# 54rt1n/shardmerge

Hardware: AMD Instinct MI355X
Metric: merged-weight GB/s per GPU + % HBM roofline, Llama-3-70B 3-way FFT merge (higher is better)
Workload: dtype f32; 1 GPU; Llama-3-70B block tensors, this rank's 1/8 slice (9 per block x 10 blocks), K=3 finetunes, bf16 in/out, resident in HBM; workload_id=llama3-70b-slice, k=3, parallelism=tensor-partition x1 (no data-path collective), streams_per_gpu=8

## Files before the change

shardmerge_amd/csrc/fft_engine.hpp:

```cpp
#pragma once
#include <cmath>
#include <cstdint>
#include <type_traits>

#if defined(__HIPCC__)
#include <hip/hip_runtime.h>
#define SM_HD __host__ __device__ __forceinline__
#else
#define SM_HD inline
#endif
#define SM_CONST static constexpr
#if defined(__HIP_DEVICE_COMPILE__)
#define SM_OPAQUE(x) asm volatile("" : "+v"(x))
#else
#define SM_OPAQUE(x) ((void)0)
#endif
#if defined(__HIP_DEVICE_COMPILE__)
#define SM_LAUNDER(x) asm("" : "+v"(x))
#else
#define SM_LAUNDER(x) ((void)0)
#endif
#if defined(__HIP_DEVICE_COMPILE__) && !defined(SM_NO_SCHED_BARRIER)
#define SM_SCHED_FENCE() __builtin_amdgcn_sched_barrier(0)
#else
// ... 548 lines not shown
                    im[i] = mk2(xi[m * R + i], xi[(m + 1) * R + i]);
                }
                if (Ns > 1) apply_twiddles<R>(re, im, tw, (j0 % Ns) * tstep, (j1 % Ns) * tstep);
                Dft<R>::run(re, im);
#pragma unroll
                for (int i = 0; i < R; ++i) {
                    xr[m * R + i] = re[i].x; xr[(m + 1) * R + i] = re[i].y;
                    xi[m * R + i] = im[i].x; xi[(m + 1) * R + i] = im[i].y;
                }
            }
        }
    } else {
#pragma unroll
        for (int m = 0; m < MB; ++m) {
            const int j = t + m * T;
            if (j < nb) {
                if (Ns > 1) {
                    const int k = j % Ns;
                    if constexpr (R <= 32 && R != 28) {
                        apply_twiddles<R>(xr + m * R, xi + m * R, tw, k * tstep, 0);
                    } else {
#pragma unroll
                        for (int i = 1; i < R; ++i) {
                            const cf2 w = tw[i * k * tstep];
                            cmul(xr[m * R + i], xi[m * R + i], w.x, w.y);
                        }
                    }
                }
                if constexpr (R == 32 && PACK == 0) DftComposite<4, 8>::run(xr + m * R, xi + m * R);
                else Dft<R>::run(xr + m * R, xi + m * R);
            }
        }
    }
}

template <int COMP, class S> SM_HD float* comp_of(S& s) { if constexpr (COMP == 0) return s.xr; else return s.xi; }

struct DynPlan { static constexpr bool is_static = false; static constexpr bool cx = false; static constexpr int waves = 4; };
template <int N_, int T_, bool CX_, int WAVES_, int... RS>
struct SPlan {
    static constexpr bool is_static = true;
    static constexpr bool cx = false;
    static constexpr int waves = WAVES_;
    static constexpr int N = N_, T = T_, npass = (int)sizeof...(RS);
    static constexpr int radix(int i) { constexpr int r[] = {RS...}; return r[i]; }
    static constexpr int ns(int p) { int v = 1; for (int i = 0; i < p; ++i) v *= radix(i); return v; }
    static constexpr int lds_floats = ((N_ + (N_ >> 5) + 1 + 31) / 32) * 32;
    static_assert(ns(npass) == N_, "radices must multiply to N");
};
template <class P> SM_HD int plan_N(const FftPlanDev& pl) { if constexpr (P::is_static) return P::N; else return pl.N; }
template <class P> SM_HD int plan_T(const FftPlanDev& pl) { if constexpr (P::is_static) return P::T; else return pl.T; }
template <class P> SM_HD int plan_lds(const FftPlanDev& pl) { if constexpr (P::is_static) return P::lds_floats; else return pl.lds_floats; }

#ifndef SM_DIAG_NOFFT
#define SM_DIAG_NOFFT 0
#endif
struct FloatPairRef { float& a; float& b; };
struct NoHook { template <class C> SM_HD void operator()(C) const {} };
template <class P, int PACK = 1, int DIAG = 0, int SKIPS = 0, class Ex, class StT, class NatScatter, class FinGather, class AfterNat = NoHook>
SM_HD void wg_fft(Ex& ex, StT& st, const FftPlanDev& pl, float* lds, NatScatter nat_scatter, FinGather fin_gather, AfterNat after_nat = AfterNat{}) {
    using S = typename StT::value_type;
    const int N = plan_N<P>(pl), T = plan_T<P>(pl), LF = plan_lds<P>(pl);
    if constexpr ((SM_DIAG_NOFFT & DIAG) != 0) {
        static_for<0, 2>([&](auto comp_c) {
            ex.each(st, [&](int tid, S& s) { nat_scatter(tid, s, comp_c); });
            ex.sync();
// ... 91 lines not shown
```

shardmerge_amd/csrc/sm_aten_core.hpp:

```cpp
#pragma once
#include <cmath>
#include <cstring>

#include "fft_engine.hpp"

namespace smhip {

SM_HD float aten_u2f(uint32_t u) { float f; memcpy(&f, &u, 4); return f; }
SM_HD uint32_t aten_f2u(float f) { uint32_t u; memcpy(&u, &f, 4); return u; }

constexpr int ATEN_LANES = 8;
constexpr int ATEN_THREADS = 256;
constexpr int ATEN_ROWS_PER_THREAD = 32;
constexpr int ATEN_CHUNK_ROWS = ATEN_THREADS * ATEN_ROWS_PER_THREAD;
constexpr int ATEN_MAX_SIGS = 16;
constexpr int ATEN_NO_EXP = -32768;

struct AtenSum { double A; uint32_t B0, B1p; };
SM_HD AtenSum aten_sum_identity() { AtenSum r; r.A = 0.0; r.B0 = 0u; r.B1p = 0u; return r; }
SM_HD AtenSum aten_sum_stop() { AtenSum r; r.A = INFINITY; r.B0 = 0u; r.B1p = 0u; return r; }
SM_HD AtenSum aten_compose(const AtenSum& l, const AtenSum& r) {
    const uint32_t pl = l.B1p >> 31, lb1 = l.B1p & 0x7fffffffu;
    const uint32_t pr = r.B1p >> 31, rb1 = r.B1p & 0x7fffffffu;
    const uint32_t mid0 = (pl ^ l.B0) & 1u, mid1 = (1u ^ pl ^ lb1) & 1u;
// ... 105 lines not shown
            constexpr int k0 = decltype(kb_c)::value * 8;
            float y[8];
#pragma unroll
            for (int k = 0; k < 8; ++k) y[k] = b[8 * (k0 + k) + ((k0 + k) >> 2)];
#pragma unroll
            for (int k = 0; k < 8; ++k) { aten_chain_add(s0, y[k]); aten_chain_add(s1, y[k]); }
            SM_SCHED_FENCE();
        });
        aten_d_of_chain(s0, ep, s.fd[0], s.fd[1]);
        aten_d_of_chain(s1, ep - 1, s.fd[2], s.fd[3]);
    });
    static_for<0, 3>([&](auto step_c) {
        constexpr int DELTA = 8 << decltype(step_c)::value;
        ex.template wave_shift_down<DELTA, 4>(st, [](S& s) { return (const uint32_t*)s.fd; }, [](S& s) { return (uint32_t*)s.fr; });
        ex.each(st, [&](int, S& s) {
            aten_d_compose(s.fd[0], s.fd[1], s.fr[0], s.fr[1]);
            aten_d_compose(s.fd[2], s.fd[3], s.fr[2], s.fr[3]);
        });
    });
    ex.each(st, [&](int tid, S& s) {
        int tid_ = tid;
        SM_OPAQUE(tid_);
        const int g = tid_ / T, t = tid_ % T;
        const int w = t >> 6, ln = t & 63;
        int sig = 0; long long mrow = 0;
        if (ln >= 8 || w >= NG || !where(g, sig, mrow)) return;
        const size_t G = (size_t)mrow * NG + w, chunk = G / ATEN_GROUPS;
        const size_t slot = ((size_t)(af.sig0 + sig) * af.nchunks + chunk) * 8 + ln;
        af.grp[(slot * 2 + 0) * ATEN_GROUPS + G % ATEN_GROUPS] = aten_sum_of_d(s.fd[0], s.fd[1]);
        af.grp[(slot * 2 + 1) * ATEN_GROUPS + G % ATEN_GROUPS] = aten_sum_of_d(s.fd[2], s.fd[3]);
    });
}

}
```

shardmerge_amd/csrc/sm_capi.inc:

```

struct smhip_ctx {
    smhip::Pipeline<SM_BACKEND> pipe;
    explicit smhip_ctx(int device) : pipe(device) {}
};

#define SM_GUARD(ctx)                      \
    if (!(ctx)) return SMHIP_ERR_ARG;      \
    (ctx)->pipe.err.clear();
#define SM_FINISH(ctx, rc)                                                        \
    do {                                                                          \
        int rc__ = (rc);                                                          \
        if (rc__ == SMHIP_OK && !(ctx)->pipe.be.ok()) {                           \
            (ctx)->pipe.err = (ctx)->pipe.be.error();                             \
            rc__ = SMHIP_ERR_HIP;                                                 \
        }                                                                         \
        return rc__;                                                              \
    } while (0)

extern "C" {

const char* smhip_version(void) { return SM_VERSION_STRING; }

int smhip_create(int device, smhip_ctx** out) {
    if (!out) return SMHIP_ERR_ARG;
// ... 170 lines not shown
    const int rc0 = ctx->pipe.reserve(1, 1);
    if (rc0) SM_FINISH(ctx, rc0);
    smhip::SigDesc sg{x, base, dtype, 1.f};
    double out = 0;
    if (!ctx->pipe.run_serial_norms(&sg, 1, n, &out))
        return ctx->pipe.fail(SMHIP_ERR_ARG, "reference_cpu norm: inputs must be 16-byte aligned");
    *norm_out = (float)out;
    SM_FINISH(ctx, SMHIP_OK);
}

int smhip_debug_option(smhip_ctx* ctx, const char* key, long value) {
    SM_GUARD(ctx);
    if (key && std::string(key) == "aten_overlap") { ctx->pipe.aten_overlap = value != 0; return SMHIP_OK; }
    if (key && std::string(key) == "emf_max_sample") { ctx->pipe.emf_max_sample = value >= 1 && value <= 4096 ? (int)value : smhip::EMF_MAX_SAMPLE; return SMHIP_OK; }
    if (key && std::string(key) == "aten_serial") { ctx->pipe.aten_serial = value != 0; return SMHIP_OK; }
    if (key && std::string(key) == "class_norms") { ctx->pipe.class_norms_mode = value >= 0 && value <= 2 ? (int)value : 1; return SMHIP_OK; }
    if (key && std::string(key) == "cand_cap") { ctx->pipe.debug_cand_cap = value > 0 ? (uint32_t)value : 0u; return SMHIP_OK; }
    if (key && std::string(key) == "sel_chunks") { ctx->pipe.debug_sel_chunks = value > 0 ? (uint32_t)value : 0u; return SMHIP_OK; }
    if (key && std::string(key) == "sel_flush_always") { ctx->pipe.debug_flush_always = value != 0; return SMHIP_OK; }
    if (key && std::string(key) == "fuse_norms") { ctx->pipe.fuse_norms = value != 0; return SMHIP_OK; }
    if (key && std::string(key) == "noise_seed") { ctx->pipe.noise_seed_base = (uint32_t)value; return SMHIP_OK; }
    if (key && std::string(key) == "spectral_intermediates") { ctx->pipe.spectral_inter = value != 0; return SMHIP_OK; }
    if (key && std::string(key) == "fuse_spec_norm") { ctx->pipe.fuse_spec_norm = value != 0; return SMHIP_OK; }
    if (key && std::string(key) == "sel_wgs_per_cu") { ctx->pipe.sel_wgs_per_cu = value > 0 ? (int)value : 5; return SMHIP_OK; }
    if (key && std::string(key) == "pair1d") { ctx->pipe.pair1d_enabled = value != 0; return SMHIP_OK; }
    if (key && std::string(key) == "spec_cull") { ctx->pipe.spec_cull = value != 0; return SMHIP_OK; }
    if (key && std::string(key) == "spec_min_bins") { ctx->pipe.spec_min_bins = value >= 0 ? (size_t)value : (size_t)1 << 20; return SMHIP_OK; }
    if (key && std::string(key) == "dftp_pairs") { ctx->pipe.dftp_pairs_enabled = value != 0; return SMHIP_OK; }
    if (key && std::string(key) == "f2s_pair") { ctx->pipe.f2s_pair = value != 0; return SMHIP_OK; }
    if (key && std::string(key) == "f1_multi") { ctx->pipe.f1_multi = value != 0; return SMHIP_OK; }
    if (key && std::string(key) == "force_bluestein") { ctx->pipe.debug_force_bluestein = value != 0; return SMHIP_OK; }
    if (key && std::string(key) == "force_split") { ctx->pipe.debug_force_split = value > 1 && value <= smhip::DFTP_MAX_P ? (int)value : 0; return SMHIP_OK; }
    if (key && std::string(key) == "fold_columns") { ctx->pipe.fold_enabled = value != 0; return SMHIP_OK; }
    if (key && std::string(key) == "fold_min_rows") { ctx->pipe.fold_min_rows = value > 0 ? (int)value : SM_FOLD_MIN_ROWS; return SMHIP_OK; }
    return ctx->pipe.fail(SMHIP_ERR_ARG, "unknown debug option");
}

int smhip_debug_query(smhip_ctx* ctx, const char* key, long* value) {
    SM_GUARD(ctx);
    if (!key || !value) return SMHIP_ERR_ARG;
    if (std::string(key) == "spec_hit") { *value = ctx->pipe.last_spec_verdict(); SM_FINISH(ctx, SMHIP_OK); }
    if (std::string(key) == "spec_checked" || std::string(key) == "spec_hits") {
        unsigned long long c = 0, h = 0;
        ctx->pipe.spec_totals(&c, &h);
        *value = (long)(std::string(key) == "spec_hits" ? h : c);
        SM_FINISH(ctx, SMHIP_OK);
    }
    if (std::string(key) == "aten_fast" || std::string(key) == "aten_group" || std::string(key) == "aten_slow") {
        unsigned long long v3[3];
        ctx->pipe.aten_stats(1, v3);
        *value = (long)v3[std::string(key) == "aten_fast" ? 0 : std::string(key) == "aten_group" ? 1 : 2];
        SM_FINISH(ctx, SMHIP_OK);
    }
    return ctx->pipe.fail(SMHIP_ERR_ARG, "unknown debug query");
}

int smhip_profile_enable(smhip_ctx* ctx, int on) { SM_GUARD(ctx); ctx->pipe.be.profile_enable(on != 0); return SMHIP_OK; }
int smhip_profile_reset(smhip_ctx* ctx) { SM_GUARD(ctx); ctx->pipe.be.profile_reset(); return SMHIP_OK; }
int smhip_profile_count(smhip_ctx* ctx) { return ctx ? ctx->pipe.be.profile_count() : 0; }
int smhip_profile_get(smhip_ctx* ctx, int i, const char** name, uint64_t* launches, double* total_ms) {
    SM_GUARD(ctx);
    return ctx->pipe.be.profile_get(i, name, launches, total_ms) ? SMHIP_OK : SMHIP_ERR_ARG;
}

}
```

shardmerge_amd/csrc/sm_kernels.hpp:

```cpp
#pragma once
#include <cmath>
#include <cstring>

#include "fft_engine.hpp"
#include "sm_aten_core.hpp"

namespace smhip {

struct cf4 { float x, y, z, w; };
struct u32x4 { uint32_t x, y, z, w; };

enum { DT_BF16 = 0, DT_F16 = 1, DT_F32 = 2 };

struct SigDesc {
    const void* x;
    const void* base;
    int dtype;
    float prescale;
};

SM_HD uint32_t umax(uint32_t a, uint32_t b) { return a > b ? a : b; }
SM_HD float u2f(uint32_t u) { float f; memcpy(&f, &u, 4); return f; }
SM_HD uint32_t f2u(float f) { uint32_t u; memcpy(&u, &f, 4); return u; }
SM_HD float bf16_to_f(uint32_t h) { return u2f(h << 16); }
// ... 160 lines not shown
    double* partials[F1_MAX_SIGS];
    long long b_off;
};
SM_HD int pick_signal(int n, int wg, int XG, int& sig) {
    sig = 0;
    if (n <= 1) return XG > 1 ? xcd_remap(wg, XG) : wg;
    const int G = XG * n;
    const int L = xcd_remap(wg, G);
    const int r = L % G;
    sig = r / XG;
    return (L / G) * XG + r % XG;
}
SM_HD int f1_pick_signal(const F1Sigs& sg, int wg, int XG, int& sig) { return pick_signal(sg.n, wg, XG, sig); }

struct F1Params {
    FftPlanDev plan;
    SigDesc a, b;
    int R, C, Cb;
    int pitch4;
    int ilv;
    int nb;
    size_t row_stride;
    int vec;
    cf4* t1;
    double* partials;
    int R2;
    int rowpair;
    int Rcol;
    size_t slab_elems;
    const cf2* twR;
    F1Sigs sigs;
    AtenFuse fuse;
    int fuse_rowpair;
};

template <class P> constexpr bool f1_full_batch() {
    if constexpr (P::is_static) return P::T <= 256; else return false;
}
#ifndef SM_ROW_PACK_MAX_T
#define SM_ROW_PACK_MAX_T 256
#endif
template <class P> constexpr bool f1_opaque() {
    if constexpr (P::is_static) return P::T >= 512; else return false;
}
#ifndef SM_ROW_PACK_BIG
#define SM_ROW_PACK_BIG 0
#endif
template <class P> constexpr int f1_pack() {
    if constexpr (P::is_static) return P::T <= SM_ROW_PACK_MAX_T ? 1 : SM_ROW_PACK_BIG; else return 1;
}

template <class P, class Ex>
SM_HD void k_f1(Ex& ex, const F1Params& p) {
    typename Ex::template State<FftState> st;
    ex.init(st);
    float* lds = ex.lds() + LDS_SCRATCH_FLOATS;
    const FftPlanDev& pl = p.plan;
    const int T = plan_T<P>(pl), C = plan_N<P>(pl);
    const int LF = plan_lds<P>(pl);
    int sig_;
    const int bid = f1_pick_signal(p.sigs, ex.bid(), (p.ilv > p.nb) ? p.ilv / p.nb : 1, sig_);
    const int pbid = p.sigs.n > 1 ? bid : ex.bid();
    SigDesc sgA = p.a, sgB = p.b;
    cf4* t1_ = p.t1;
    double* partials_ = p.partials;
    if (p.sigs.n > 1) {
// ... 206 lines not shown
                    if (comp == 0) { o[2 * u] = 0.5f * (v1 + v2); o[2 * u + 1] = 0.5f * (v2 - v1); }
                    else           { o[2 * u] = 0.5f * (v1 - v2); o[2 * u + 1] = 0.5f * (v1 + v2); }
                    if (!sgB.x) o[2 * u + 1] = 0.f;
                }
            }
        },
        [&](auto comp_c) {
            constexpr int comp = decltype(comp_c)::value;
            if constexpr (P::is_static) {
                if constexpr (aten_fusable(P::N, P::T)) {
                    if (p.fuse.prefix)
                        aten_fused_rows<P::N, P::T>(ex, st, p.fuse, lds, LF, fuse_where(comp), [](FftState& s) { return s.fep[comp]; });
                }
            }
        });

    ex.each(st, [&](int tid, FftState& s) {
        int tid_ = tid;
        if constexpr (f1_opaque<P>()) SM_OPAQUE(tid_);
        const int g = tid_ / T, t = tid_ % T;
        const int row = bid * p.nb + g;
        if (row >= p.R) return;
        cf4* dst = t1_ + (size_t)(row / p.ilv) * p.pitch4 * p.ilv + (row % p.ilv);
#pragma unroll
        for (int u = 0; u < EMAX / 2 + 1; ++u) {
            const int k = t + u * T;
            if (k < p.Cb) {
                cf4 v;
                v.x = s.xr[2 * u]; v.y = s.xi[2 * u]; v.z = s.xi[2 * u + 1]; v.w = s.xr[2 * u + 1];
                dst[(size_t)k * p.ilv] = v;
            }
        }
    });
}

#ifndef SM_F1Q_QB
#define SM_F1Q_QB 1
#endif
#ifndef SM_F1Q_PREFETCH_B
#define SM_F1Q_PREFETCH_B 1
#endif
#ifndef SM_F1Q_PACK
#define SM_F1Q_PACK 1
#endif
template <class P> constexpr bool f1q_eligible() {
    if constexpr (P::is_static) return 4 * P::T <= 1024 && (P::N / P::T) % 2 == 0 && P::N % 8 == 0; else return false;
}

struct F1QState {
    float xr[EREG];
    float xi[EREG];
    double red[4];
    u32x4 rb[EMAX / 8], rbb[EMAX / 8];
};

template <class P, class Ex>
SM_HD void k_f1q(Ex& ex, const F1Params& p) {
    if constexpr (!f1q_eligible<P>()) { return; } else {
    typename Ex::template State<F1QState> st;
    ex.init(st);
    float* lds = ex.lds() + LDS_SCRATCH_FLOATS;
    const FftPlanDev& pl = p.plan;
    constexpr int T = P::T, C = P::N, LF = P::lds_floats;
    constexpr int E2 = C / T / 2;
    constexpr int NJ = (E2 + 3) / 4;
    constexpr int NQ = EMAX / 8;
// ... 3395 lines not shown
```

shardmerge_amd/csrc/sm_pipeline.hpp:

```cpp
#pragma once
#include <algorithm>
#include <cmath>
#include <cstdio>
#include <map>
#include <string>
#include <vector>

#include "../../include/shardmerge_hip.h"
#include "sm_kernels.hpp"
#include "sm_aten_norm.hpp"
#include "sm_bluestein.hpp"
#include "sm_lora.hpp"

namespace smhip {

#define SM_KERNEL_TAG(Tag, ParamsT, NAME, CALL)                                      \
    struct Tag {                                                                     \
        using Params = ParamsT;                                                      \
        static constexpr int waves = 4;                                              \
        static constexpr int max_threads = 1024;                                     \
        static const char* name() { return NAME; }                                   \
        template <class Ex> static SM_HD void run(Ex& ex, const Params& p) { CALL; } \
    };
#define SM_KERNEL_TAG_LB(Tag, ParamsT, NAME, CALL, MAXT, WAVES)                      \
    struct Tag {                                                                     \
        using Params = ParamsT;                                                      \
        static constexpr int waves = WAVES;                                          \
        static constexpr int max_threads = MAXT;                                     \
        static const char* name() { return NAME; }                                   \
        template <class Ex> static SM_HD void run(Ex& ex, const Params& p) { CALL; } \
    };
template <class P, int GROUPS> constexpr int fft_max_threads() {
    if constexpr (P::is_static) return (GROUPS * P::T < 256) ? 256 : (GROUPS * P::T > 1024 ? 1024 : GROUPS * P::T);
    else return 1024;
}
#ifndef SM_W3_MAX_THREADS
#define SM_W3_MAX_THREADS 256
#endif
#define SM_FFT_KERNEL_TAG(Tag, ParamsT, NAME, CALL, GROUPS, WAVES)                   \
    template <class P> struct Tag {                                                  \
        using Params = ParamsT;                                                      \
        static constexpr int waves = (WAVES < 4 && P::is_static && fft_max_threads<P, GROUPS>() <= SM_W3_MAX_THREADS) ? WAVES : 4; \
        static constexpr int max_threads = waves < 4 ? fft_max_threads<P, GROUPS>() : 1024; \
        static const char* name() { return NAME; }                                   \
        template <class Ex> static SM_HD void run(Ex& ex, const Params& p) { CALL; } \
    };
SM_FFT_KERNEL_TAG(KF1, F1Params, "f1_rows_fwd", k_f1<P>(ex, p), 1, 3)
SM_FFT_KERNEL_TAG(KF2, F2Params, "f2_cols_fwd", (k_f2<P, f2_bins<P>()>(ex, p)), 2 * f2_bins<P>(), 4)
SM_FFT_KERNEL_TAG(KI1x1, I1Params, "i1_cols_inv", (k_i1<P, 1>(ex, p)), 1, 4)
SM_FFT_KERNEL_TAG(KI1x2, I1Params, "i1_cols_inv", (k_i1<P, i1_bins<P>()>(ex, p)), i1_bins<P>(), 4)
SM_FFT_KERNEL_TAG(KI2, I2Params, "i2_rows_inv", k_i2<P>(ex, p), 1, 4)
SM_FFT_KERNEL_TAG(KF2S, F2SParams, "f2s_cols_fwd1", (k_f2s<P, f2s_groups<P>()>(ex, p)), f2s_groups<P>(), 4)
SM_FFT_KERNEL_TAG(KF1Q, F1Params, "f1_rows_fwd", k_f1q<P>(ex, p), 4, 4)
SM_FFT_KERNEL_TAG(KF2Q, F2Params, "f2_cols_fwd", (k_f2<P, f2_bins<P>(), true>(ex, p)), 2 * f2_bins<P>(), 4)
SM_FFT_KERNEL_TAG(KF2SQ, F2SParams, "f2s_cols_fwd1", (k_f2s<P, f2s_groups<P>(), true>(ex, p)), f2s_groups<P>(), 4)
SM_FFT_KERNEL_TAG(KI1x1Q, I1Params, "i1_cols_inv", (k_i1<P, 1, true>(ex, p)), 1, 4)
SM_FFT_KERNEL_TAG(KI1x2Q, I1Params, "i1_cols_inv", (k_i1<P, i1_bins<P>(), true>(ex, p)), i1_bins<P>(), 4)
#define SM_BLUE_KERNEL_TAG(Tag, ParamsT, NAME, CALL)                                 \
    template <class P> struct Tag {                                                  \
        using Params = ParamsT;                                                      \
        static constexpr int max_threads = fft_max_threads<P, 1>();                  \
        static constexpr int waves = max_threads > 512 ? 4 : 2;                      \
        static const char* name() { return NAME; }                                   \
        template <class Ex> static SM_HD void run(Ex& ex, const Params& p) { CALL; } \
    };
SM_BLUE_KERNEL_TAG(KF1B, F1BParams, "f1_rows_fwd", k_f1b<P>(ex, p))
SM_BLUE_KERNEL_TAG(KI2B, I2BParams, "i2_rows_inv", k_i2b<P>(ex, p))
SM_FFT_KERNEL_TAG(KPair1d, Pair1dParams, "pair_1d", k_pair1d<P>(ex, p), 1, 1)

#ifndef SM_COLS_MAX_THREADS
#define SM_COLS_MAX_THREADS 1024
#endif
#ifndef SM_F2_MAX_THREADS
#define SM_F2_MAX_THREADS 512
#endif
#ifndef SM_R14336
#define SM_R14336 16, 16, 8, 7
#endif
#ifndef SM_R7168
#define SM_R7168 32, 32, 7
#endif
#ifndef SM_T8192
#define SM_T8192 256
#define SM_W8192 4
#define SM_R8192 32, 16, 16
#endif
// ... 510 lines not shown
            for (int j = 0; j < N; ++j) {
                const double ang = -2.0 * M_PI * (double)j / (double)N;
                tw[j].x = (float)cos(ang); tw[j].y = (float)sin(ang);
            }
            void* d = be.alloc(sizeof(cf2) * N);
            if (!d) return fail(SMHIP_ERR_NOMEM, "twiddle alloc failed");
            be.h2d(d, tw.data(), sizeof(cf2) * N, stream);
            be.sync(stream);
            it = rough_tw_.emplace(N, d).first;
        }
        *out = (const cf2*)it->second;
        return SMHIP_OK;
    }
    int run_dftp(const Geo& g, void* buf, bool rowpair, int ilv, int pitch, size_t slice_stride, bool inverse) {
        DftpParams q;
        int rc = rough_twiddles(g.R * g.rough, &q.tw);
        if (rc) return rc;
        q.buf = (cf4*)buf; q.p = g.rough; q.M = g.R; q.units = rowpair ? g.R / 2 : g.R; q.rowpair = rowpair ? 1 : 0;
        q.ilv = ilv; q.pitch = pitch; q.ncols = g.C / 2 + 1; q.slice_stride = slice_stride; q.inverse = inverse ? 1 : 0;
        q.cols = DFTP_COLS;
        if (q.p <= DFTP_PAIR_MAX_P && dftp_pairs_enabled) {
            q.cols = dftp_pairs_cols(q.p);
            const int ntp = (q.ncols + q.cols - 1) / q.cols;
            const size_t ldsp = LDS_SCRATCH_FLOATS * 4 + dftp_pairs_lds_bytes(q.p) + ((size_t)(q.p / 2 + 1) + 64) * sizeof(cf2);
            be.template launch<KDftpPairs>((q.units + DFTP_UNITS - 1) / DFTP_UNITS * ntp, 256, ldsp, q, stream);
            return SMHIP_OK;
        }
        const int ntiles = (q.ncols + DFTP_COLS - 1) / DFTP_COLS;
        const size_t lds = LDS_SCRATCH_FLOATS * 4 + (size_t)q.p * DFTP_COLS * sizeof(cf4) + (size_t)q.p * sizeof(cf2);
        be.template launch<KDftp>(q.units * ntiles, 256, lds, q, stream);
        return SMHIP_OK;
    }

    int run_f1(const Geo& g, const SigDesc& a, const SigDesc& b, int& grid_out) {
        F1Params p;
        bool blue; BluesteinTab bt;
        int rc = get_row_plan(g.C, p.plan, blue, bt);
        if (rc) return rc;
        p.a = a; p.b = b; p.R = g.R; p.C = g.C; p.Cb = g.C / 2 + 1; p.pitch4 = g.pitch4; p.ilv = g.ilv;
        p.sigs.n = 0;
        p.fuse.prefix = nullptr; p.fuse.grp = nullptr; p.fuse.nchunks = 0; p.fuse.sig0 = 0; p.fuse_rowpair = 0;
        p.nb = blue ? 1 : std::max(1, 256 / p.plan.T);
        p.row_stride = (size_t)g.C;
        p.vec = !blue && (g.C % 8 == 0) && aligned16(a.x) && aligned16(a.base) && aligned16(b.x) && aligned16(b.base);
        if (fused_.armed && p.vec && g.batch == 1 && g.rough == 1) { p.fuse = fused_.af; p.fuse_rowpair = 0; fused_.used = true; }
        p.t1 = (cf4*)t1_.p;
        p.partials = d_part();
        p.R2 = 0; p.rowpair = 0; p.Rcol = g.R; p.twR = nullptr; p.slab_elems = fold_slab_elems(g);
        if (g.fold == 4) {
            if (!p.vec) return fail(SMHIP_ERR_ARG, "internal: folded row pass on unaligned input");
            FftPlanDev colp;
            if ((rc = get_plan(g.R, colp))) return rc;
            p.R2 = g.R / 4; p.twR = colp.tw; p.ilv = FOLD_ILV; p.nb = 4;
            const int gridq = (int)round_up((size_t)p.R2, 8 * p.ilv);
            if ((size_t)gridq * 2 > PART_DOUBLES) return fail(SMHIP_ERR_SHAPE, "too many rows");
            launch_fft<KF1Q>(p.plan, gridq, 4 * p.plan.T, (LDS_SCRATCH_FLOATS + (size_t)4 * p.plan.lds_floats) * 4, p);
            grid_out = gridq;
            return SMHIP_OK;
        }
        const int xg = p.ilv > p.nb ? p.ilv / p.nb : 1;
        const bool joint = joint_rows(g);
        const int nlaunch = joint ? 1 : g.batch;
        if (joint) p.R = g.R * g.rough;
        const int grid = (int)round_up((size_t)(p.R + p.nb - 1) / p.nb, 8 * xg);
        if ((size_t)grid * 2 * nlaunch > PART_DOUBLES) return fail(SMHIP_ERR_SHAPE, "too many rows");
        const size_t lds = (LDS_SCRATCH_FLOATS + (size_t)p.nb * p.plan.lds_floats) * 4;
        for (int bi = 0; bi < nlaunch; ++bi) {
            p.a = sig_at(a, (size_t)bi * g.R * g.C); p.b = sig_at(b, (size_t)bi * g.R * g.C);
            p.t1 = (cf4*)t1_.p + (size_t)bi * g.t1_slice;
            p.partials = d_part() + (size_t)bi * 2 * grid;
            if (blue) { F1BParams q; q.f = p; q.bt = bt; launch_fft<KF1B>(p.plan, grid, p.plan.T, lds, q); }
            else launch_fft<KF1>(p.plan, grid, p.nb * p.plan.T, lds, p, p.vec != 0);
        }
        grid_out = grid * nlaunch;
        if (g.rough > 1) return run_dftp(g, t1_.p, false, p.ilv, g.pitch4, g.t1_slice, false);
        return SMHIP_OK;
    }
    static size_t dt_size(int dt) { return dt == DT_F32 ? 4 : 2; }
    static SigDesc sig_at(const SigDesc& s, size_t elems) {
        SigDesc r = s;
        if (r.x) r.x = (const char*)r.x + elems * dt_size(s.dtype);
        if (r.base) r.base = (const char*)r.base + elems * dt_size(s.dtype);
        return r;
    }
    static size_t fold_slab_elems(const Geo& g, bool rowpair = false) {
        return round_up((size_t)g.R / (rowpair ? 8 : 4), 8) * (size_t)g.pitch4;
    }
    static bool joint_rows(const Geo& g) { return g.rough > 1 && g.R % 16 == 0; }
    int run_f1_rowpairs(const Geo& g, const SigDesc& sig, void* t1buf = nullptr, double* partials = nullptr, int* grid_out = nullptr,
                        F1Sigs* multi = nullptr) {
        F1Params p;
        bool blue; BluesteinTab bt;
        int rc = get_row_plan(g.C, p.plan, blue, bt);
        if (rc) return rc;
        SigDesc a = sig, b = sig;
        b.x = (const char*)sig.x + (size_t)g.C * dt_size(sig.dtype);
        if (sig.base) b.base = (const char*)sig.base + (size_t)g.C * dt_size(sig.dtype);
        p.a = a; p.b = b; p.R = g.R / 2; p.C = g.C; p.Cb = g.C / 2 + 1; p.pitch4 = g.pitch4; p.ilv = F2S_ILV;
        p.sigs.n = 0;
        p.fuse.prefix = nullptr; p.fuse.grp = nullptr; p.fuse.nchunks = 0; p.fuse.sig0 = 0; p.fuse_rowpair = 0;
        const int nm = multi ? multi->n : 1;
        if (multi && (blue || nm < 2 || nm > F1_MAX_SIGS)) return SMHIP_ERR_ARG;
        p.nb = blue ? 1 : std::max(1, 256 / p.plan.T);
        p.row_stride = (size_t)2 * g.C;
        p.vec = !blue && (g.C % 8 == 0) && aligned16(a.x) && aligned16(a.base) && aligned16(b.x) && aligned16(b.base);
        if (fused_.armed && p.vec && g.batch == 1 && g.rough == 1) {
            p.fuse = fused_.af; p.fuse.sig0 = multi ? 0 : fused_.next_sig; p.fuse_rowpair = 1; fused_.used = true;
        }
        p.t1 = (cf4*)(t1buf ? t1buf : t1_.p);
        p.partials = partials ? partials : d_part();
        p.R2 = 0; p.rowpair = 0; p.Rcol = g.R; p.twR = nullptr; p.slab_elems = fold_slab_elems(g, true);
        if (g.fold == 4) {
            if (!p.vec) return fail(SMHIP_ERR_ARG, "internal: folded row pass on unaligned input");
            FftPlanDev colp;
            if ((rc = get_plan(g.R, colp))) return rc;
            p.R2 = g.R / 8; p.rowpair = 1; p.twR = colp.tw; p.ilv = F2S_ILV; p.nb = 4;
            const int gridq = (int)round_up((size_t)p.R2, 8 * p.ilv);
            if (multi) {
                if ((size_t)gridq * 2 * nm > PART_DOUBLES) return SMHIP_ERR_ARG;
                for (int i = 0; i < nm; ++i) multi->partials[i] = p.partials + (size_t)i * 2 * gridq;
                multi->b_off = (long long)((size_t)g.C * dt_size(sig.dtype));
                p.sigs = *multi;
            }
            launch_fft<KF1Q>(p.plan, gridq * nm, 4 * p.plan.T, (LDS_SCRATCH_FLOATS + (size_t)4 * p.plan.lds_floats) * 4, p);
            if (grid_out) *grid_out = gridq;
            return SMHIP_OK;
        }
        const int xgs = p.ilv > p.nb ? p.ilv / p.nb : 1;
        const bool joint = joint_rows(g);
        const int nlaunch = joint ? 1 : g.batch;
        if (joint) p.R = g.R * g.rough / 2;
        const int grid = (int)round_up((size_t)(p.R + p.nb - 1) / p.nb, 8 * xgs);
        if (multi && (nlaunch != 1 || g.rough > 1 || (size_t)grid * 2 * nm > PART_DOUBLES || !p.vec)) return SMHIP_ERR_ARG;
        if ((size_t)grid * 2 * nlaunch > PART_DOUBLES) return fail(SMHIP_ERR_SHAPE, "too many rows");
        const size_t lds = (LDS_SCRATCH_FLOATS + (size_t)p.nb * p.plan.lds_floats) * 4;
        cf4* const t1base = p.t1;
        double* const pbase = p.partials;
        if (multi) {
            for (int i = 0; i < nm; ++i) multi->partials[i] = pbase + (size_t)i * 2 * grid;
            multi->b_off = (long long)((size_t)g.C * dt_size(sig.dtype));
            p.sigs = *multi;
            launch_fft<KF1>(p.plan, grid * nm, p.nb * p.plan.T, lds, p, true);
            if (grid_out) *grid_out = grid;
            return SMHIP_OK;
        }
        for (int bi = 0; bi < nlaunch; ++bi) {
            p.a = sig_at(a, (size_t)bi * g.R * g.C); p.b = sig_at(b, (size_t)bi * g.R * g.C);
            p.t1 = t1base + (size_t)bi * (g.t1_slice / 2);
            p.partials = pbase + (size_t)bi * 2 * grid;
            if (blue) { F1BParams q; q.f = p; q.bt = bt; launch_fft<KF1B>(p.plan, grid, p.plan.T, lds, q); }
            else launch_fft<KF1>(p.plan, grid, p.nb * p.plan.T, lds, p, p.vec != 0);
        }
        if (grid_out) *grid_out = grid * nlaunch;
        if (g.rough > 1) return run_dftp(g, t1base, true, F2S_ILV, g.pitch4, g.t1_slice / 2, false);
        return SMHIP_OK;
    }
    struct F2SSecond { const void* t1; bool role_a; float scale; };
    int run_f2s(const Geo& g, bool role_a, float scale, bool hist, const void* t1buf = nullptr, int* im_parts = nullptr,
                const F2SSecond* second = nullptr) {
        F2SParams p;
        p.two = 0; p.t1_2 = nullptr; p.role_a_2 = 0; p.scale_2 = 0.f; p.re_2 = nullptr;
        if (second) {
            if (g.batch != 1 || second->role_a == role_a) return fail(SMHIP_ERR_ARG, "internal: paired column pass");
            p.two = 1; p.t1_2 = (const cf4*)second->t1; p.role_a_2 = second->role_a ? 1 : 0; p.scale_2 = second->scale;
            p.re_2 = plane(g, second->role_a ? P_REA : P_REB);
        }
        const int nsg = second ? 2 : 1;
        const int Rt = g.R / g.fold;
        int rc = get_plan(Rt, p.plan);
        if (rc) return rc;
        p.t1 = (const cf4*)(t1buf ? t1buf : t1_.p); p.pitch4 = g.pitch4 * g.fold; p.R = Rt; p.C = g.C;
        p.Cb = g.fold == 4 ? 4 * g.pitch4 : g.C / 2 + 1;
        p.slab = g.pitch4; p.Cb_real = g.C / 2 + 1; p.Rfull = g.R; p.slab_elems = fold_slab_elems(g, true);
        p.role_a = role_a ? 1 : 0; p.scale = scale;
        p.re = plane(g, role_a ? P_REA : P_REB); p.im = plane(g, P_IMA);
        p.hist = hist ? d_hist() : nullptr;
        const bool st = is_static_plan(p.plan);
        const int G = st ? (f2_nsig_for(p.plan.T) == 2 ? 2 * f2_bins_for(p.plan.T, p.plan.N) : 1) : 1;
        const int xg = G >= 8 ? 1 : 8 / G;
        const int grid = (int)round_up((size_t)(p.Cb + G - 1) / G, 8 * xg) * nsg;
        const size_t lds = (LDS_SCRATCH_FLOATS + (size_t)G * p.plan.lds_floats + HIST1_BINS) * 4;
        const bool any_a = role_a || (second && second->role_a);
        const bool want_im = im_parts && any_a && (size_t)grid * g.batch <= PART_IM_DOUBLES;
        if (im_parts) *im_parts = want_im ? grid * g.batch : -1;
// ... 1547 lines not shown
```

shardmerge_amd/csrc/smhip_device.hpp:

```cpp
#pragma once
#include <hip/hip_runtime.h>

#include "sm_pipeline.hpp"

namespace smhip {

struct DeviceExec {
    template <class S> struct State { using value_type = S; S s; };
    __device__ __forceinline__ int bid() const { return blockIdx.x; }
    __device__ __forceinline__ int nthreads() const { return blockDim.x; }
    __device__ __forceinline__ int nblocks() const { return gridDim.x; }
    __device__ __forceinline__ float* lds() {
        extern __shared__ __attribute__((aligned(16))) float sm_dyn_lds[];
        return sm_dyn_lds;
    }
    template <class S> __device__ __forceinline__ void init(State<S>&) {}
    template <class S, class F> __device__ __forceinline__ void each(State<S>& st, F&& f) { f((int)threadIdx.x, st.s); }
    __device__ __forceinline__ void sync() { __syncthreads(); }
    __device__ __forceinline__ void lds_atomic_add(uint32_t* p, uint32_t v) { atomicAdd(p, v); }
    __device__ __forceinline__ uint32_t lds_atomic_add_ret(uint32_t* p, uint32_t v) { return atomicAdd(p, v); }
    __device__ __forceinline__ uint32_t global_atomic_add_ret_u32(uint32_t* p, uint32_t v) { return atomicAdd(p, v); }
    __device__ __forceinline__ void global_atomic_add(unsigned long long* p, unsigned long long v) { atomicAdd(p, v); }
    __device__ __forceinline__ void global_atomic_add_u32(uint32_t* p, uint32_t v) { atomicAdd(p, v); }
    __device__ __forceinline__ void global_atomic_or_u32(uint32_t* p, uint32_t v) { atomicOr(p, v); }
// ... 27 lines not shown
            for (int q = 0; q < NV; ++q) v[q] += __shfl_down(v[q], off, 64);
        }
        double* scratch = (double*)lds();
        const int wave = threadIdx.x >> 6, lane = threadIdx.x & 63;
        const int nw = (blockDim.x + 63) >> 6;
        if (lane == 0) {
#pragma unroll
            for (int q = 0; q < NV; ++q) scratch[wave * NV + q] = v[q];
        }
        __syncthreads();
        if (threadIdx.x == 0) {
            double tot[NV];
#pragma unroll
            for (int q = 0; q < NV; ++q) tot[q] = 0.0;
            for (int w = 0; w < nw; ++w) {
#pragma unroll
                for (int q = 0; q < NV; ++q) tot[q] += scratch[w * NV + q];
            }
            f((const double*)tot);
        }
        __syncthreads();
    }
};

template <class K>
__global__ void __launch_bounds__(K::max_threads, K::waves) sm_kernel(const typename K::Params p) {
    DeviceExec ex;
    K::run(ex, p);
}

#define SM_FFT_KERNELS_OF(X, ...)                      \
    X(KF1<__VA_ARGS__>) X(KF2<__VA_ARGS__>) X(KI1x1<__VA_ARGS__>) X(KI1x2<__VA_ARGS__>) X(KI2<__VA_ARGS__>) X(KF2S<__VA_ARGS__>) \
    X(KF1Q<__VA_ARGS__>) X(KF2Q<__VA_ARGS__>) X(KF2SQ<__VA_ARGS__>) X(KI1x1Q<__VA_ARGS__>) X(KI1x2Q<__VA_ARGS__>) \
    X(KPair1d<__VA_ARGS__>) X(KF1B<__VA_ARGS__>) X(KI2B<__VA_ARGS__>)

}
```

shardmerge_amd/csrc/smhip_side.hip:

```cpp
#include "smhip_device.hpp"

namespace smhip {
#define SM_INST(...) template __global__ void sm_kernel<__VA_ARGS__>(const typename __VA_ARGS__::Params);
#if SM_SIDE_GROUP == 0
SM_SIDE_KERNELS_0(SM_INST)
#elif SM_SIDE_GROUP == 1
SM_SIDE_KERNELS_1(SM_INST)
#elif SM_SIDE_GROUP == 2
SM_SIDE_KERNELS_2(SM_INST)
#elif SM_SIDE_GROUP == 3
SM_INST(KF1<DynPlan>) SM_INST(KF1Q<DynPlan>) SM_INST(KI2<DynPlan>) SM_INST(KPair1d<DynPlan>)
#elif SM_SIDE_GROUP == 4
SM_INST(KF2<DynPlan>) SM_INST(KF2Q<DynPlan>) SM_INST(KF2S<DynPlan>) SM_INST(KF2SQ<DynPlan>)
#elif SM_SIDE_GROUP == 5
SM_INST(KI1x1<DynPlan>) SM_INST(KI1x2<DynPlan>) SM_INST(KI1x1Q<DynPlan>) SM_INST(KI1x2Q<DynPlan>)
#elif SM_SIDE_GROUP == 6
SM_INST(KF1B<DynPlan>) SM_INST(KI2B<DynPlan>)
#else
#error "SM_SIDE_GROUP must be 0..6"
#endif
}
```

Before: 86.32 GB/s.

## Compute real row FFTs via half-length complex FFT with post-combine

Adds a KF1H row-forward kernel that packs a real row of length C=28672 as a complex signal of length C/2, runs the half-size FFT, then separates even and odd parts and applies twiddles to produce the full spectrum. The fused norm accumulation is reworked for the new layout. Each real row previously went through a full-size complex FFT with zero imaginary part, which wasted arithmetic and LDS traffic. The path is gated to one row width and a static 512-thread plan, adds an extra gather and combine step, and brings a new kernel with its own register pressure.

```diff
diff --git a/shardmerge_amd/csrc/fft_engine.hpp b/shardmerge_amd/csrc/fft_engine.hpp
--- a/shardmerge_amd/csrc/fft_engine.hpp
+++ b/shardmerge_amd/csrc/fft_engine.hpp
@@ -604,6 +604,19 @@
             }
         }
     }
+}
+
+template <int COMP>
+SM_HD void rh_fwd_gather(const float* l, int M, int k, float& a, float& b) {
+    const int k2 = (k == 0) ? 0 : M - k;
+    const float v1 = l[lpad(k)], v2 = l[lpad(k2)];
+    if (COMP == 0) { a = 0.5f * (v1 + v2); b = 0.5f * (v2 - v1); }
+    else           { a = 0.5f * (v1 - v2); b = 0.5f * (v1 + v2); }
+}
+SM_HD void rh_fwd_combine(float er, float ei, float orr, float oi, cf2 w, cf2& xk, cf2& xmk) {
+    const float pr = w.x * orr - w.y * oi, pi = w.x * oi + w.y * orr;
+    xk.x = er + pr; xk.y = ei + pi;
+    xmk.x = er - pr; xmk.y = pi - ei;
 }
 
 template <int COMP, class S> SM_HD float* comp_of(S& s) { if constexpr (COMP == 0) return s.xr; else return s.xi; }
diff --git a/shardmerge_amd/csrc/sm_aten_core.hpp b/shardmerge_amd/csrc/sm_aten_core.hpp
--- a/shardmerge_amd/csrc/sm_aten_core.hpp
+++ b/shardmerge_amd/csrc/sm_aten_core.hpp
@@ -161,4 +161,62 @@
     });
 }
 
-}
+SM_HD constexpr bool aten_fusable_rh(int C, int T) {
+    return SM_FUSE_NORMS && C % (8 * ATEN_GROUP_ROWS) == 0 && 32 * (C / (8 * ATEN_GROUP_ROWS)) <= T;
+}
+template <int C>
+SM_HD int aten_fused_ep_rh(const AtenFuse& af, int t, int comp, int sig, long long mrow) {
+    constexpr int NG = C / (8 * ATEN_GROUP_ROWS);
+    const int w = t >> 5, c = 2 * (t & 3) + comp;
+    if (w >= NG) return ATEN_NO_EXP;
+    const size_t G = (size_t)mrow * NG + w, chunk = G / ATEN_GROUPS;
+    const size_t slot = ((size_t)(af.sig0 + sig) * af.nchunks + chunk) * 8 + c;
+    return aten_exp_of(af.prefix[slot] * (1.0 + ATEN_LEAD_MARGIN));
+}
+template <int C, int COMP, class Ex, class StT, class EpOf>
+SM_HD void aten_fused_rows_rh(Ex& ex, StT& st, const AtenFuse& af, const float* lds, int sig, long long mrow, EpOf ep_of) {
+    using S = typename StT::value_type;
+    constexpr int NG = C / (8 * ATEN_GROUP_ROWS);
+    ex.each(st, [&](int tid, S& s) {
+        int tid_ = tid;
+        SM_OPAQUE(tid_);
+        const int w = tid_ >> 5, ln = tid_ & 31, c = ln & 3, run = ln >> 2;
+        s.fd[0] = 0u; s.fd[1] = 0u; s.fd[2] = 0u; s.fd[3] = 0u;
+        const int ep = ep_of(s);
+        if (w >= NG || ep == ATEN_NO_EXP) return;
+        vf2 s0 = aten_chain_start(ep), s1 = aten_chain_start(ep - 1);
+        const int p0 = 4 * (ATEN_GROUP_ROWS * w + ATEN_ROWS_PER_THREAD * run) + c;
+        const float* b = lds + lpad(p0);
+        static_for<0, ATEN_ROWS_PER_THREAD / 8>([&](auto kb_c) {
+            constexpr int k0 = decltype(kb_c)::value * 8;
+            float y[8];
+#pragma unroll
+            for (int k = 0; k < 8; ++k) y[k] = b[4 * (k0 + k) + ((k0 + k) >> 3)];
+#pragma unroll
+            for (int k = 0; k < 8; ++k) { aten_chain_add(s0, y[k]); aten_chain_add(s1, y[k]); }
+            SM_SCHED_FENCE();
+        });
+        aten_d_of_chain(s0, ep, s.fd[0], s.fd[1]);
+        aten_d_of_chain(s1, ep - 1, s.fd[2], s.fd[3]);
+    });
+    static_for<0, 3>([&](auto step_c) {
+        constexpr int DELTA = 4 << decltype(step_c)::value;
+        ex.template wave_shift_down<DELTA, 4>(st, [](S& s) { return (const uint32_t*)s.fd; }, [](S& s) { return (uint32_t*)s.fr; });
+        ex.each(st, [&](int, S& s) {
+            aten_d_compose(s.fd[0], s.fd[1], s.fr[0], s.fr[1]);
+            aten_d_compose(s.fd[2], s.fd[3], s.fr[2], s.fr[3]);
+        });
+    });
+    ex.each(st, [&](int tid, S& s) {
+        int tid_ = tid;
+        SM_OPAQUE(tid_);
+        const int w = tid_ >> 5, ln = tid_ & 31;
+        if (ln >= 4 || w >= NG) return;
+        const size_t G = (size_t)mrow * NG + w, chunk = G / ATEN_GROUPS;
+        const size_t slot = ((size_t)(af.sig0 + sig) * af.nchunks + chunk) * 8 + 2 * ln + COMP;
+        af.grp[(slot * 2 + 0) * ATEN_GROUPS + G % ATEN_GROUPS] = aten_sum_of_d(s.fd[0], s.fd[1]);
+        af.grp[(slot * 2 + 1) * ATEN_GROUPS + G % ATEN_GROUPS] = aten_sum_of_d(s.fd[2], s.fd[3]);
+    });
+}
+
+}
diff --git a/shardmerge_amd/csrc/sm_capi.inc b/shardmerge_amd/csrc/sm_capi.inc
--- a/shardmerge_amd/csrc/sm_capi.inc
+++ b/shardmerge_amd/csrc/sm_capi.inc
@@ -226,6 +226,7 @@
     if (key && std::string(key) == "force_bluestein") { ctx->pipe.debug_force_bluestein = value != 0; return SMHIP_OK; }
     if (key && std::string(key) == "force_split") { ctx->pipe.debug_force_split = value > 1 && value <= smhip::DFTP_MAX_P ? (int)value : 0; return SMHIP_OK; }
     if (key && std::string(key) == "fold_columns") { ctx->pipe.fold_enabled = value != 0; return SMHIP_OK; }
+    if (key && std::string(key) == "row_real_half") { ctx->pipe.row_real_half = value != 0; return SMHIP_OK; }
     if (key && std::string(key) == "fold_min_rows") { ctx->pipe.fold_min_rows = value > 0 ? (int)value : SM_FOLD_MIN_ROWS; return SMHIP_OK; }
     return ctx->pipe.fail(SMHIP_ERR_ARG, "unknown debug option");
 }
@@ -233,6 +234,7 @@
 int smhip_debug_query(smhip_ctx* ctx, const char* key, long* value) {
     SM_GUARD(ctx);
     if (!key || !value) return SMHIP_ERR_ARG;
+    if (std::string(key) == "row_real_half_launches") { *value = (long)ctx->pipe.f1h_launches; SM_FINISH(ctx, SMHIP_OK); }
     if (std::string(key) == "spec_hit") { *value = ctx->pipe.last_spec_verdict(); SM_FINISH(ctx, SMHIP_OK); }
     if (std::string(key) == "spec_checked" || std::string(key) == "spec_hits") {
         unsigned long long c = 0, h = 0;
diff --git a/shardmerge_amd/csrc/sm_kernels.hpp b/shardmerge_amd/csrc/sm_kernels.hpp
--- a/shardmerge_amd/csrc/sm_kernels.hpp
+++ b/shardmerge_amd/csrc/sm_kernels.hpp
@@ -216,6 +216,7 @@
     F1Sigs sigs;
     AtenFuse fuse;
     int fuse_rowpair;
+    const cf2* twC;
 };
 
 template <class P> constexpr bool f1_full_batch() {
@@ -488,6 +489,160 @@
             }
         }
     });
+}
+
+template <class P> constexpr bool f1h_eligible() {
+    if constexpr (P::is_static) return P::T == 512 && P::N % (4 * P::T) == 0 && (P::N / 2) % P::T == 0; else return false;
+}
+
+template <class P, class Ex>
+SM_HD void k_f1h(Ex& ex, const F1Params& p) {
+    if constexpr (!f1h_eligible<P>()) { return; } else {
+    typename Ex::template State<FftState> st;
+    ex.init(st);
+    float* lds = ex.lds() + LDS_SCRATCH_FLOATS;
+    const FftPlanDev& pl = p.plan;
+    constexpr int T = P::T, M = P::N, C = 2 * M;
+    constexpr int NQ = M / (4 * T);
+    constexpr int NU = M / 2 / T + 1;
+    static_assert(4 * NQ <= EREG && 2 * NU <= EREG, "register slots");
+    int sig_;
+    const int hb = f1_pick_signal(p.sigs, ex.bid(), 2 * (p.ilv > 1 ? p.ilv : 1), sig_);
+    const int unit = hb >> 1, half = hb & 1;
+    SigDesc sg = half ? p.b : p.a;
+    cf4* t1_ = p.t1;
+    double* partials_ = p.partials;
+    if (p.sigs.n > 1) {
+        const long long off = half ? p.sigs.b_off : 0;
+        sg.x = (const char*)p.sigs.x[sig_] + off;
+        sg.base = p.sigs.base[sig_] ? (const char*)p.sigs.base[sig_] + off : nullptr;
+        t1_ = p.sigs.t1[sig_]; partials_ = p.sigs.partials[sig_];
+    }
+    cf2* const dst = (cf2*)(t1_ + (size_t)(unit / p.ilv) * p.pitch4 * p.ilv + unit % p.ilv) + half;
+    const size_t kstep = 2 * (size_t)p.ilv;
+    if (unit >= p.R || !sg.x) {
+        ex.each(st, [&](int tid, FftState&) {
+            if (tid == 0) partials_[2 * (size_t)unit + half] = 0.0;
+            if (unit < p.R)
+                for (int k = tid; k <= M; k += T) dst[(size_t)k * kstep] = cf2{0.f, 0.f};
+        });
+        return;
+    }
+    const int fsig = p.fuse_rowpair ? sig_ : half;
+    const long long fmrow = p.fuse_rowpair ? 2LL * unit + half : (long long)unit;
+    if constexpr (aten_fusable_rh(C, T)) {
+        if (p.fuse.prefix) ex.each(st, [&](int tid, FftState& s) {
+            s.fep[0] = aten_fused_ep_rh<C>(p.fuse, tid, 0, fsig, fmrow);
+            s.fep[1] = aten_fused_ep_rh<C>(p.fuse, tid, 1, fsig, fmrow);
+        });
+    }
+
+    ex.each(st, [&](int tid, FftState& s) {
+        const bool has_base = sg.base != nullptr;
+        const size_t row0 = (size_t)unit * p.row_stride / 8;
+        double ss = 0.0;
+        auto batches = [&](auto qb_c, auto load) {
+            constexpr int QB = decltype(qb_c)::value;
+            static_for<0, (NQ + QB - 1) / QB>([&](auto h_c) {
+                constexpr int Q0 = decltype(h_c)::value * QB, Q1 = (Q0 + QB < NQ) ? Q0 + QB : NQ;
+                float v[QB][8], b[QB][8];
+                load(std::integral_constant<int, Q0>{}, std::integral_constant<int, Q1>{}, v, b);
+#pragma unroll
+                for (int q = Q0; q < Q1; ++q) {
+                    float x[8], ps = 0.f;
+#pragma unroll
+                    for (int c = 0; c < 8; ++c) {
+                        x[c] = (v[q - Q0][c] - (has_base ? b[q - Q0][c] : 0.f)) * sg.prescale;
+                        ps += x[c] * x[c];
+                    }
+#pragma unroll
+                    for (int j = 0; j < 4; ++j) { s.xr[4 * q + j] = x[2 * j]; s.xi[4 * q + j] = x[2 * j + 1]; }
+                    ss += ps;
+                }
+            });
+        };
+        if (sg.dtype != DT_F32) {
+            const u32x4* px = (const u32x4*)sg.x;
+            const u32x4* pb = has_base ? (const u32x4*)sg.base : px;
+            batches(std::integral_constant<int, 4>{}, [&](auto q0_c, auto q1_c, float (*v)[8], float (*b)[8]) {
+                constexpr int Q0 = decltype(q0_c)::value, Q1 = decltype(q1_c)::value;
+                u32x4 r[Q1 - Q0], rb[Q1 - Q0];
+#pragma unroll
+                for (int q = Q0; q < Q1; ++q) r[q - Q0] = px[row0 + tid + q * T];
+#pragma unroll
+                for (int q = Q0; q < Q1; ++q) rb[q - Q0] = pb[row0 + tid + q * T];
+#pragma unroll
+                for (int q = Q0; q < Q1; ++q) { decode16x8(r[q - Q0], sg.dtype, v[q - Q0]); decode16x8(rb[q - Q0], sg.dtype, b[q - Q0]); }
+            });
+        } else {
+            const cf4* px = (const cf4*)sg.x;
+            const cf4* pb = has_base ? (const cf4*)sg.base : px;
+            batches(std::integral_constant<int, 2>{}, [&](auto q0_c, auto q1_c, float (*v)[8], float (*b)[8]) {
+                constexpr int Q0 = decltype(q0_c)::value, Q1 = decltype(q1_c)::value;
+                cf4 r[Q1 - Q0][2], rb[Q1 - Q0][2];
+#pragma unroll
+                for (int q = Q0; q < Q1; ++q) { r[q - Q0][0] = px[2 * (row0 + tid + q * T)]; r[q - Q0][1] = px[2 * (row0 + tid + q * T) + 1]; }
+#pragma unroll
+                for (int q = Q0; q < Q1; ++q) { rb[q - Q0][0] = pb[2 * (row0 + tid + q * T)]; rb[q - Q0][1] = pb[2 * (row0 + tid + q * T) + 1]; }
+#pragma unroll
+                for (int q = Q0; q < Q1; ++q) {
+                    const cf4 x0 = r[q - Q0][0], x1 = r[q - Q0][1], b0 = rb[q - Q0][0], b1 = rb[q - Q0][1];
+                    v[q - Q0][0] = x0.x; v[q - Q0][1] = x0.y; v[q - Q0][2] = x0.z; v[q - Q0][3] = x0.w;
+                    v[q - Q0][4] = x1.x; v[q - Q0][5] = x1.y; v[q - Q0][6] = x1.z; v[q - Q0][7] = x1.w;
+                    b[q - Q0][0] = b0.x; b[q - Q0][1] = b0.y; b[q - Q0][2] = b0.z; b[q - Q0][3] = b0.w;
+                    b[q - Q0][4] = b1.x; b[q - Q0][5] = b1.y; b[q - Q0][6] = b1.z; b[q - Q0][7] = b1.w;
+                }
+            });
+        }
+        s.red[0] = ss;
+    });
+    ex.template block_sum<1>(st, [&](const double* tot) { partials_[2 * (size_t)unit + half] = tot[0]; });
+
+    wg_fft<P, f1_pack<P>(), 1>(ex, st, pl, lds,
+        [&](int tid, FftState& s, auto comp_c) {
+            constexpr int comp = decltype(comp_c)::value;
+            const float* x = comp_of<comp>(s);
+#pragma unroll
+            for (int q = 0; q < NQ; ++q) {
+                float* b = lds + lpad(4 * (tid + q * T));
+#pragma unroll
+                for (int j = 0; j < 4; ++j) b[j] = x[4 * q + j];
+            }
+        },
+        [&](int tid, FftState& s, auto comp_c) {
+            constexpr int comp = decltype(comp_c)::value;
+            int tid_ = tid;
+            SM_OPAQUE(tid_);
+            float* o = comp_of<comp>(s);
+#pragma unroll
+            for (int u = 0; u < NU; ++u) {
+                const int k = tid_ + u * T;
+                if (k <= M / 2) rh_fwd_gather<comp>(lds, M, k, o[2 * u], o[2 * u + 1]);
+            }
+        },
+        [&](auto comp_c) {
+            constexpr int comp = decltype(comp_c)::value;
+            if constexpr (aten_fusable_rh(C, T)) {
+                if (p.fuse.prefix)
+                    aten_fused_rows_rh<C, comp>(ex, st, p.fuse, lds, fsig, fmrow, [](FftState& s) { return s.fep[comp]; });
+            }
+        });
+
+    ex.each(st, [&](int tid, FftState& s) {
+        int tid_ = tid;
+        SM_OPAQUE(tid_);
+#pragma unroll
+        for (int u = 0; u < NU; ++u) {
+            const int k = tid_ + u * T;
+            if (k <= M / 2) {
+                cf2 xk, xmk;
+                rh_fwd_combine(s.xr[2 * u], s.xi[2 * u], s.xi[2 * u + 1], s.xr[2 * u + 1], p.twC[k], xk, xmk);
+                dst[(size_t)k * kstep] = xk;
+                if (2 * k != M) dst[(size_t)(M - k) * kstep] = xmk;
+            }
+        }
+    });
+    }
 }
 
 #ifndef SM_F1Q_QB
diff --git a/shardmerge_amd/csrc/sm_pipeline.hpp b/shardmerge_amd/csrc/sm_pipeline.hpp
--- a/shardmerge_amd/csrc/sm_pipeline.hpp
+++ b/shardmerge_amd/csrc/sm_pipeline.hpp
@@ -52,6 +52,7 @@
 SM_FFT_KERNEL_TAG(KI2, I2Params, "i2_rows_inv", k_i2<P>(ex, p), 1, 4)
 SM_FFT_KERNEL_TAG(KF2S, F2SParams, "f2s_cols_fwd1", (k_f2s<P, f2s_groups<P>()>(ex, p)), f2s_groups<P>(), 4)
 SM_FFT_KERNEL_TAG(KF1Q, F1Params, "f1_rows_fwd", k_f1q<P>(ex, p), 4, 4)
+SM_FFT_KERNEL_TAG(KF1H, F1Params, "f1_rows_fwd", k_f1h<P>(ex, p), 1, 4)
 SM_FFT_KERNEL_TAG(KF2Q, F2Params, "f2_cols_fwd", (k_f2<P, f2_bins<P>(), true>(ex, p)), 2 * f2_bins<P>(), 4)
 SM_FFT_KERNEL_TAG(KF2SQ, F2SParams, "f2s_cols_fwd1", (k_f2s<P, f2s_groups<P>(), true>(ex, p)), f2s_groups<P>(), 4)
 SM_FFT_KERNEL_TAG(KI1x1Q, I1Params, "i1_cols_inv", (k_i1<P, 1, true>(ex, p)), 1, 4)
@@ -628,6 +629,27 @@
         return SMHIP_OK;
     }
 
+    bool row_real_half = true;
+    unsigned long long f1h_launches = 0;
+    bool f1_real_half(const F1Params& p, bool blue) const {
+        return row_real_half && !blue && p.vec && p.nb == 1 && p.C == 28672;
+    }
+    int launch_f1(F1Params p, int grid, bool blue, bool allow_static) {
+        if (f1_real_half(p, blue)) {
+            FftPlanDev hp;
+            const int rc = get_plan(p.C / 2, hp);
+            if (rc) return rc;
+            if (is_static_plan(hp) && hp.T == 512) {
+                p.twC = p.plan.tw; p.plan = hp;
+                launch_fft<KF1H>(hp, 2 * grid, hp.T, (LDS_SCRATCH_FLOATS + (size_t)hp.lds_floats) * 4, p);
+                ++f1h_launches;
+                return SMHIP_OK;
+            }
+        }
+        launch_fft<KF1>(p.plan, grid, p.nb * p.plan.T, (LDS_SCRATCH_FLOATS + (size_t)p.nb * p.plan.lds_floats) * 4, p, allow_static);
+        return SMHIP_OK;
+    }
+
     int run_f1(const Geo& g, const SigDesc& a, const SigDesc& b, int& grid_out) {
         F1Params p;
         bool blue; BluesteinTab bt;
@@ -642,7 +664,7 @@
         if (fused_.armed && p.vec && g.batch == 1 && g.rough == 1) { p.fuse = fused_.af; p.fuse_rowpair = 0; fused_.used = true; }
         p.t1 = (cf4*)t1_.p;
         p.partials = d_part();
-        p.R2 = 0; p.rowpair = 0; p.Rcol = g.R; p.twR = nullptr; p.slab_elems = fold_slab_elems(g);
+        p.R2 = 0; p.rowpair = 0; p.Rcol = g.R; p.twR = nullptr; p.twC = nullptr; p.slab_elems = fold_slab_elems(g);
         if (g.fold == 4) {
             if (!p.vec) return fail(SMHIP_ERR_ARG, "internal: folded row pass on unaligned input");
             FftPlanDev colp;
@@ -666,7 +688,7 @@
             p.t1 = (cf4*)t1_.p + (size_t)bi * g.t1_slice;
             p.partials = d_part() + (size_t)bi * 2 * grid;
             if (blue) { F1BParams q; q.f = p; q.bt = bt; launch_fft<KF1B>(p.plan, grid, p.plan.T, lds, q); }
-            else launch_fft<KF1>(p.plan, grid, p.nb * p.plan.T, lds, p, p.vec != 0);
+            else if ((rc = launch_f1(p, grid, blue, p.vec != 0))) return rc;
         }
         grid_out = grid * nlaunch;
         if (g.rough > 1) return run_dftp(g, t1_.p, false, p.ilv, g.pitch4, g.t1_slice, false);
@@ -705,7 +727,7 @@
         }
         p.t1 = (cf4*)(t1buf ? t1buf : t1_.p);
         p.partials = partials ? partials : d_part();
-        p.R2 = 0; p.rowpair = 0; p.Rcol = g.R; p.twR = nullptr; p.slab_elems = fold_slab_elems(g, true);
+        p.R2 = 0; p.rowpair = 0; p.Rcol = g.R; p.twR = nullptr; p.twC = nullptr; p.slab_elems = fold_slab_elems(g, true);
         if (g.fold == 4) {
             if (!p.vec) return fail(SMHIP_ERR_ARG, "internal: folded row pass on unaligned input");
             FftPlanDev colp;
@@ -736,7 +758,7 @@
             for (int i = 0; i < nm; ++i) multi->partials[i] = pbase + (size_t)i * 2 * grid;
             multi->b_off = (long long)((size_t)g.C * dt_size(sig.dtype));
             p.sigs = *multi;
-            launch_fft<KF1>(p.plan, grid * nm, p.nb * p.plan.T, lds, p, true);
+            if ((rc = launch_f1(p, grid * nm, blue, true))) return rc;
             if (grid_out) *grid_out = grid;
             return SMHIP_OK;
         }
@@ -745,7 +767,7 @@
             p.t1 = t1base + (size_t)bi * (g.t1_slice / 2);
             p.partials = pbase + (size_t)bi * 2 * grid;
             if (blue) { F1BParams q; q.f = p; q.bt = bt; launch_fft<KF1B>(p.plan, grid, p.plan.T, lds, q); }
-            else launch_fft<KF1>(p.plan, grid, p.nb * p.plan.T, lds, p, p.vec != 0);
+            else if ((rc = launch_f1(p, grid, blue, p.vec != 0))) return rc;
         }
         if (grid_out) *grid_out = grid * nlaunch;
         if (g.rough > 1) return run_dftp(g, t1base, true, F2S_ILV, g.pitch4, g.t1_slice / 2, false);
diff --git a/shardmerge_amd/csrc/smhip_device.hpp b/shardmerge_amd/csrc/smhip_device.hpp
--- a/shardmerge_amd/csrc/smhip_device.hpp
+++ b/shardmerge_amd/csrc/smhip_device.hpp
@@ -83,6 +83,6 @@
 #define SM_FFT_KERNELS_OF(X, ...)                      \
     X(KF1<__VA_ARGS__>) X(KF2<__VA_ARGS__>) X(KI1x1<__VA_ARGS__>) X(KI1x2<__VA_ARGS__>) X(KI2<__VA_ARGS__>) X(KF2S<__VA_ARGS__>) \
     X(KF1Q<__VA_ARGS__>) X(KF2Q<__VA_ARGS__>) X(KF2SQ<__VA_ARGS__>) X(KI1x1Q<__VA_ARGS__>) X(KI1x2Q<__VA_ARGS__>) \
-    X(KPair1d<__VA_ARGS__>) X(KF1B<__VA_ARGS__>) X(KI2B<__VA_ARGS__>)
+    X(KPair1d<__VA_ARGS__>) X(KF1B<__VA_ARGS__>) X(KI2B<__VA_ARGS__>) X(KF1H<__VA_ARGS__>)
 
 }
diff --git a/shardmerge_amd/csrc/smhip_side.hip b/shardmerge_amd/csrc/smhip_side.hip
--- a/shardmerge_amd/csrc/smhip_side.hip
+++ b/shardmerge_amd/csrc/smhip_side.hip
@@ -9,7 +9,7 @@
 #elif SM_SIDE_GROUP == 2
 SM_SIDE_KERNELS_2(SM_INST)
 #elif SM_SIDE_GROUP == 3
-SM_INST(KF1<DynPlan>) SM_INST(KF1Q<DynPlan>) SM_INST(KI2<DynPlan>) SM_INST(KPair1d<DynPlan>)
+SM_INST(KF1<DynPlan>) SM_INST(KF1Q<DynPlan>) SM_INST(KI2<DynPlan>) SM_INST(KPair1d<DynPlan>) SM_INST(KF1H<DynPlan>)
 #elif SM_SIDE_GROUP == 4
 SM_INST(KF2<DynPlan>) SM_INST(KF2Q<DynPlan>) SM_INST(KF2S<DynPlan>) SM_INST(KF2SQ<DynPlan>)
 #elif SM_SIDE_GROUP == 5
```

Result: no change. 86.40 GB/s, median of 4 (+0.1%).
